# rueberger/MJHMC

Hardware: AMD Instinct MI355X
Metric: particle-steps/sec (ndims x nparticles x L) (higher is better)
Workload: dtype f64 state (ProductOfT: around the f32 matrix-core force)

## Files before the change

### mjhmc_amd/csrc/dense_pot64.hip

```cpp
#include <hip/hip_runtime.h>
#include <stdint.h>

#include <algorithm>

#include "dense_pot.hpp"
#include "dense_pot64_kernels.hpp"
#include "dense_pot_tile.hpp"

namespace mjhmc {

__global__ void pot64_cold_list_kernel(const double* __restrict__ Hflf_in, const double* __restrict__ Hspec_in, int64_t N,
                                       int* __restrict__ list, int* __restrict__ count, const Control* ctl) {
  if (ctl->failed) return;
  const int64_t p = (int64_t)blockIdx.x * blockDim.x + threadIdx.x;
  const double hc = p < N ? Hflf_in[p] : 0.0, hs = p < N ? Hspec_in[p] : 0.0;
  append_cold(list, count, (p < N) && !(hc == hc) && !(hs == hs), p);
}

template <int NB, bool REPLAY, int MODE>
__global__ __launch_bounds__(256, 1) void pot64_jump_kernel(const Pot64JumpArgs a, const PotModel mdl) {
  const PotExperts xp;
#include "dense_pot64_jump.inc"
}

// ... 37 lines not shown
      if (k != 0) {
        a.EX_out[p] = EX0;
        a.EV_out[p] = EV0;
      }
      a.Hflf_out[p] = k == 0 ? H0 : __builtin_nan("");
      a.Hspec_out[p] = k == 1 ? HL : __builtin_nan("");
    }
    __syncthreads();
    if (__syncthreads_or(sh.s.move[c] != 0)) {
      const size_t roff = (size_t)p * (128 * NB) + 32 * NB * w + 4 * NB * h;
      VTile<NB> v;
      Tile<NB> g;
      pot64_finish<NB, REPLAY, kModeMJHMC, true>(a, sh, p, alive, roff, w, c, h, v, g);
      __syncthreads();
    }
  }
  if (any_bad) {
    a.ctl->failed = 1;
    a.ctl->failed_iter = a.iter;
  }
  __shared__ unsigned tally[4];
  if (threadIdx.x < 4) tally[threadIdx.x] = 0;
  __syncthreads();
  if (n0) atomicAdd(&tally[0], n0);
  if (n1) atomicAdd(&tally[1], n1);
  if (n2) atomicAdd(&tally[2], n2);
  if (n3) atomicAdd(&tally[3], n3);
  __syncthreads();
  if (threadIdx.x < 4 && tally[threadIdx.x]) atomicAdd(&a.stats[threadIdx.x], (unsigned long long)tally[threadIdx.x]);
}

static int resident_cus64() {
  int dev = 0, cus = 0;
  (void)hipGetDevice(&dev);
  (void)hipDeviceGetAttribute(&cus, hipDeviceAttributeMultiprocessorCount, dev);
  return std::max(1, cus);
}

int pot64_scratch_workgroups() { return resident_cus64(); }

template <int NB, int MODE>
static void launch64_mode(const Pot64JumpArgs& a, const PotModel& mdl, unsigned grid, hipStream_t st, const PotGenerated* gen) {
  const bool replay = MODE == kModeControl ? (a.runif && a.noise) : (a.rexp && a.noise);
  if (gen) pot_launch_generated(gen->jump64[MODE][replay ? 1 : 0], grid, st, a, mdl, gen->lin);
  else if (replay) hipLaunchKernelGGL((pot64_jump_kernel<NB, true, MODE>), dim3(grid), dim3(256), 0, st, a, mdl);
  else hipLaunchKernelGGL((pot64_jump_kernel<NB, false, MODE>), dim3(grid), dim3(256), 0, st, a, mdl);
}

template <int NB>
static void launch64_nb(const Pot64JumpArgs& a, const PotModel& mdl, hipStream_t st, const PotGenerated* gen) {
  const int cus = resident_cus64();
  if (a.mode == kModeMJHMC) {
    if (a.iter == 0 || a.rescan) {
      (void)hipMemsetAsync(std::min(a.cold_count, std::min(a.next_count, a.zero_count)), 0, 3 * sizeof(int), st);
      hipLaunchKernelGGL(pot64_cold_list_kernel, dim3((unsigned)((a.N + 255) / 256)), dim3(256), 0, st, a.Hflf_in, a.Hspec_in,
                         a.N, a.cold_list, a.cold_count, (const Control*)a.ctl);
    }
    const unsigned grid = (unsigned)std::min<int64_t>(2 * a.ntiles, cus);
    launch64_mode<NB, kModeMJHMC>(a, mdl, grid, st, gen);
    const unsigned fgrid = (unsigned)std::min<int64_t>(a.ntiles, 4 * cus);
    if (a.rexp && a.noise) hipLaunchKernelGGL((pot64_decide_kernel<NB, true>), dim3(fgrid), dim3(256), 0, st, a);
    else hipLaunchKernelGGL((pot64_decide_kernel<NB, false>), dim3(fgrid), dim3(256), 0, st, a);
  } else {
    const unsigned grid = (unsigned)std::min<int64_t>(a.ntiles, cus);
    if (a.mode == kModeCT) launch64_mode<NB, kModeCT>(a, mdl, grid, st, gen);
    else launch64_mode<NB, kModeControl>(a, mdl, grid, st, gen);
  }
}

void pot64_launch_jump(const Pot64JumpArgs& a, const PotModel& mdl, hipStream_t st, const PotGenerated* gen) {
  if (mdl.dim == 128) launch64_nb<1>(a, mdl, st, gen);
  else if (mdl.dim == 256) launch64_nb<2>(a, mdl, st, gen);
  else launch64_nb<4>(a, mdl, st, gen);
}

#ifdef POT_STAMPS
}
extern "C" int mjhmc_pot64_stamps(unsigned long long* out) {
  return (int)hipMemcpyFromSymbol(out, HIP_SYMBOL(mjhmc::g_pot_stamp), sizeof(mjhmc::g_pot_stamp));
}
extern "C" int mjhmc_pot64_item_stamps(unsigned long long* out) {
  return (int)hipMemcpyFromSymbol(out, HIP_SYMBOL(mjhmc::g_pot_istamp), sizeof(mjhmc::g_pot_istamp));
}
namespace mjhmc {
#endif

}
```

### mjhmc_amd/csrc/dense_pot64_jump.inc

```
  __shared__ Shared64<NB> sh;
  if (a.ctl->failed) return;
  const int lane = threadIdx.x & 63, w = threadIdx.x >> 6, c = lane & 31, h = lane >> 5;
  const int ncold = MODE == kModeMJHMC ? *a.cold_count : 0;
  const int64_t nft = (ncold + kP - 1) / kP;
  if ((int64_t)blockIdx.x >= nft + a.ntiles) return;
  if (MODE == kModeMJHMC && blockIdx.x == 0 && threadIdx.x == 0) {
    *a.zero_count = 0;
    if (ncold) atomicAdd(&a.stats[3], (unsigned long long)ncold << 32);
  }
  __shared__ unsigned tally[5];
  if (threadIdx.x < 5) tally[threadIdx.x] = 0;
  AReg<NB> ar;
  areg_load<NB>(mdl, w, c, h, ar);
  stage_bias<NB>(mdl, sh.s);
  const Work<NB> wk = work_of<NB>(a.scratch, blockIdx.x, w, lane);
  for (int64_t item = blockIdx.x; item < nft + a.ntiles; item += gridDim.x) {
    const bool inverse = item < nft;
    [[maybe_unused]] const int istamp_item = (int)(item / gridDim.x) & 15;
    auto column_of = [&](int64_t it) -> int64_t {
      if (it < nft) {
        const int64_t slot = it * kP + c;
        return a.cold_list[slot < ncold ? slot : ncold - 1];
      }
      return (it - nft) * kP + c;
    };
    Tile<NB> g;
    VTile<NB> v;
    float exl = 0.f;
    double EVL;
    {
      const int64_t p = column_of(item);
      POT_ISTAMP(0);
      staged_start<NB>(sh.s, wk, a.X_in, a.V_in, a.G_in, p, w, c, h, g, v, inverse);
      POT_ISTAMP(1);
      EVL = pot64_trajectory<NB>(mdl, xp, ar, sh, w, c, h, lane, wk, g, v, a.L, a.eps, a.chalf, &exl);
      POT_ISTAMP(2);
    }
    int64_t item_again = item;
    asm volatile("" : "+s"(item_again));
    const int64_t p = column_of(item_again);
    const bool alive = p < a.N;
    const size_t roff = (size_t)p * (128 * NB) + 32 * NB * w + 4 * NB * h;
    if (!inverse) staged_end_x<NB>(sh.s, wk, a.X_out, p, w, c, h);
    POT_ISTAMP(3);
    const double EXL = (double)exl;
    const double HL = EXL + EVL;
    if (inverse) {
      if (w == 0 && h == 0) a.Hwork[p] = HL;
      __syncthreads();
      POT_ISTAMP(4);
      continue;
    }

    if constexpr (MODE == kModeMJHMC) {
      if (w == 0 && h == 0) {
        a.EX_out[p] = EXL;
        a.EV_out[p] = EVL;
      }
      staged_end_vg<NB>(sh.s, a.V_out, a.G_out, p, w, c, h, v, g);
      POT_ISTAMP(4);
      continue;
    }

    if (w == 0 && h == 0) {
      const int64_t pp = alive ? p : 0;
      const uint32_t pid = (uint32_t)(a.first_pid + pp);
      const double EX0 = a.EX_in[p], EV0 = a.EV_in[p];
      const double H0 = EX0 + EV0;
      double best = 0.0;
      bool bad = false, gate = false;
      const int k = pot64_decide<REPLAY, MODE>(a, H0, HL, 0.0, pp, pid, best, bad, gate);
      if (bad && alive) tally[4] = 1;
      a.dwell[p] = best;
      a.dwell_ring[p] = best;
      a.trans[p] = (uint8_t)k;
      sh.s.move[c] = k | (gate ? 4 : 0);
      {
        unsigned long long b0, b1, b2, b3 = 0ull;
        if constexpr (MODE == kModeControl) {
          b0 = __ballot(alive && k == 3);
          b1 = __ballot(alive && k == 2);
          b2 = __ballot(alive && gate);
          b3 = __ballot(alive && k == 1);
        } else {
          b0 = __ballot(alive && k == 0);
          b1 = __ballot(alive && k == 1);
          b2 = __ballot(alive && k == 2);
        }
        if (c == 0) {
          if (b0) atomicAdd(&tally[0], (unsigned)__popcll(b0));
          if (b1) atomicAdd(&tally[1], (unsigned)__popcll(b1));
          if (b2) atomicAdd(&tally[2], (unsigned)__popcll(b2));
          if (b3) atomicAdd(&tally[3], (unsigned)__popcll(b3));
        }
      }
      const bool took_L = MODE == kModeControl ? (k & 1) : (k == 0);
      a.EX_out[p] = took_L ? EXL : EX0;
      a.EV_out[p] = took_L ? EVL : EV0;
      a.Hflf_out[p] = __builtin_nan("");
    }
    __syncthreads();
    pot64_finish<NB, REPLAY, MODE, false>(a, sh, p, alive, roff, w, c, h, v, g);
    __syncthreads();
    POT_ISTAMP(4);
  }
  __syncthreads();
  if (threadIdx.x == 0 && tally[4]) {
    a.ctl->failed = 1;
    a.ctl->failed_iter = a.iter;
  }
  if (threadIdx.x < 4 && tally[threadIdx.x]) atomicAdd(&a.stats[threadIdx.x], (unsigned long long)tally[threadIdx.x]);
```

### mjhmc_amd/csrc/dense_pot64_kernels.hpp

```cpp
#pragma once
#ifndef __HIPCC_RTC__
#include <hip/hip_runtime.h>
#endif
#include <stdint.h>

#include "dense_pot.hpp"
#include "dense_pot_tile.hpp"

namespace mjhmc {

template <int NB>
struct DVecN;
template <>
struct DVecN<1> {
  using type = double;
};
template <>
struct DVecN<2> {
  using type = __attribute__((ext_vector_type(2))) double;
};
template <>
struct DVecN<4> {
  using type = __attribute__((ext_vector_type(4))) double;
};
// ... 31 lines not shown
template <int NB>
struct Shared64 {
  Shared<NB> s;
  double red64[4][kP];
  double zn[128 * NB];
  f32x4 park[kPark / 2][256];
};

template <int NB>
struct Work {
  static constexpr int PB = NB == 1 ? 8 : 16;
  static constexpr int PQ = NB * 8 / PB;
  static constexpr unsigned kArea = 16u * PQ * 64u * PB;
  __amdgpu_buffer_rsrc_t rs;
  unsigned voff;
  static constexpr unsigned xb = 0;
  static constexpr unsigned vb = 4 * kArea;
};
template <int NB>
__device__ __forceinline__ Work<NB> work_of(double* scratch, unsigned wg, int w, int lane) {
  Work<NB> k;
  char* base = (char*)scratch + (size_t)wg * (8 * Work<NB>::kArea);
  k.rs = __builtin_amdgcn_make_buffer_rsrc((void*)base, 0, 8 * Work<NB>::kArea, 0x00020000);
  k.voff = (unsigned)w * Work<NB>::kArea + (unsigned)lane * Work<NB>::PB;
  return k;
}
using uvec4 = __attribute__((ext_vector_type(4))) unsigned;
using uvec2 = __attribute__((ext_vector_type(2))) unsigned;
using f64x2 = __attribute__((ext_vector_type(2))) double;
template <int NB>
__device__ __forceinline__ typename DVecN<NB>::type wk_load(const Work<NB>& k, unsigned area, int q) {
  if constexpr (NB == 1) {
    return __builtin_bit_cast(double, __builtin_amdgcn_raw_buffer_load_b64(k.rs, k.voff, area + (unsigned)q * 512u, 0));
  } else if constexpr (NB == 2) {
    return __builtin_bit_cast(f64x2, __builtin_amdgcn_raw_buffer_load_b128(k.rs, k.voff, area + (unsigned)q * 1024u, 0));
  } else {
    const f64x2 lo = __builtin_bit_cast(f64x2, __builtin_amdgcn_raw_buffer_load_b128(k.rs, k.voff, area + (unsigned)q * 2048u, 0));
    const f64x2 hi = __builtin_bit_cast(f64x2, __builtin_amdgcn_raw_buffer_load_b128(k.rs, k.voff, area + (unsigned)q * 2048u + 1024u, 0));
    typename DVecN<4>::type v;
    v[0] = lo[0];
    v[1] = lo[1];
    v[2] = hi[0];
    v[3] = hi[1];
    return v;
  }
}
template <int NB>
__device__ __forceinline__ void wk_store(const Work<NB>& k, unsigned area, int q, const typename DVecN<NB>::type& v) {
  if constexpr (NB == 1) {
    __builtin_amdgcn_raw_buffer_store_b64(__builtin_bit_cast(uvec2, v), k.rs, k.voff, area + (unsigned)q * 512u, 0);
  } else if constexpr (NB == 2) {
    __builtin_amdgcn_raw_buffer_store_b128(__builtin_bit_cast(uvec4, v), k.rs, k.voff, area + (unsigned)q * 1024u, 0);
  } else {
    f64x2 lo, hi;
    lo[0] = v[0];
    lo[1] = v[1];
    hi[0] = v[2];
    hi[1] = v[3];
    __builtin_amdgcn_raw_buffer_store_b128(__builtin_bit_cast(uvec4, lo), k.rs, k.voff, area + (unsigned)q * 2048u, 0);
    __builtin_amdgcn_raw_buffer_store_b128(__builtin_bit_cast(uvec4, hi), k.rs, k.voff, area + (unsigned)q * 2048u + 1024u, 0);
  }
}

template <int NB>
struct PieceOf {
  using type = uvec4;
};
template <>
struct PieceOf<1> {
  using type = unsigned long long;
};
template <int NB>
struct Stage {
  using P = typename PieceOf<NB>::type;
  static constexpr int PB = sizeof(P);
  static constexpr int RB = 1024 * NB;
  static constexpr int RP = RB / PB;
  static constexpr int K = 32 * RP / 256;
  static constexpr int KB = K < 16 ? K : 16;
};
__device__ __forceinline__ unsigned stage_addr(int row, int piece, int pb, int rb) {
  return (unsigned)(row * rb + ((piece ^ (row & 15)) * pb));
}
template <int NB>
__device__ __forceinline__ void stage_rows_in(const double* rows, int64_t p, char* img) {
  using S = Stage<NB>;
  using P = typename S::P;
  const int t = threadIdx.x;
#pragma unroll 1
  for (int i0 = 0; i0 < S::K; i0 += S::KB) {
    P buf[S::KB];
#pragma unroll
    for (int i = 0; i < S::KB; ++i) {
      const int k = (i0 + i) * 256 + t, row = k / S::RP, piece = k % S::RP;
      const int64_t pr = __shfl((long long)p, row);
      buf[i] = *reinterpret_cast<const P*>(reinterpret_cast<const char*>(rows) + (size_t)pr * S::RB + (size_t)piece * S::PB);
    }
#pragma unroll
    for (int i = 0; i < S::KB; ++i) {
      const int k = (i0 + i) * 256 + t, row = k / S::RP, piece = k % S::RP;
      *reinterpret_cast<P*>(img + stage_addr(row, piece, S::PB, S::RB)) = buf[i];
    }
  }
}
template <int NB>
__device__ __forceinline__ void stage_rows_out(double* rows, int64_t p, const char* img) {
  using S = Stage<NB>;
  using P = typename S::P;
  const int t = threadIdx.x;
#pragma unroll 1
  for (int i0 = 0; i0 < S::K; i0 += S::KB) {
#pragma unroll
    for (int i = 0; i < S::KB; ++i) {
      const int k = (i0 + i) * 256 + t, row = k / S::RP, piece = k % S::RP;
      const int64_t pr = __shfl((long long)p, row);
      *reinterpret_cast<P*>(reinterpret_cast<char*>(rows) + (size_t)pr * S::RB + (size_t)piece * S::PB) =
          *reinterpret_cast<const P*>(img + stage_addr(row, piece, S::PB, S::RB));
    }
  }
}
template <int NB>
__device__ __forceinline__ typename DVecN<NB>::type stage_get(const char* img, int w, int c, int h, int q) {
  using S = Stage<NB>;
  const int first = (8 * NB * (32 * w + acc_row(q, h))) / S::PB;
  if constexpr (NB == 4) {
    const f64x2 lo = *reinterpret_cast<const f64x2*>(img + stage_addr(c, first, S::PB, S::RB));
    const f64x2 hi = *reinterpret_cast<const f64x2*>(img + stage_addr(c, first + 1, S::PB, S::RB));
    typename DVecN<4>::type v;
    v[0] = lo[0];
    v[1] = lo[1];
    v[2] = hi[0];
    v[3] = hi[1];
    return v;
  } else {
    return *reinterpret_cast<const typename DVecN<NB>::type*>(img + stage_addr(c, first, S::PB, S::RB));
  }
}
template <int NB>
__device__ __forceinline__ void stage_put(char* img, int w, int c, int h, int q, const typename DVecN<NB>::type& v) {
  using S = Stage<NB>;
  const int first = (8 * NB * (32 * w + acc_row(q, h))) / S::PB;
  if constexpr (NB == 4) {
    f64x2 lo, hi;
    lo[0] = v[0];
    lo[1] = v[1];
    hi[0] = v[2];
    hi[1] = v[3];
    *reinterpret_cast<f64x2*>(img + stage_addr(c, first, S::PB, S::RB)) = lo;
    *reinterpret_cast<f64x2*>(img + stage_addr(c, first + 1, S::PB, S::RB)) = hi;
  } else {
    *reinterpret_cast<typename DVecN<NB>::type*>(img + stage_addr(c, first, S::PB, S::RB)) = v;
  }
}
template <int NB>
__device__ __forceinline__ char* stage_image(Shared<NB>& s) {
  static_assert(sizeof(s.pub) == 32 * Stage<NB>::RB, "the staging image is the two B-operand images");
  return reinterpret_cast<char*>(&s.pub[0][0]);
}

template <int NB>
struct VTile {
  double b[NB][16];
};

template <int NB, int NKICK>
__device__ __forceinline__ void kick_drift_pass(const Work<NB>& wk, const Tile<NB>& g, VTile<NB>& v, double c, double eps,
                                                PubWave<NB>* pub0, int w, int lane) {
  using DV = typename DVecN<NB>::type;
  DV xa[4], xb[4];
  auto load4 = [&](int q4, DV(&x)[4]) {
#pragma unroll
    for (int qq = 0; qq < 4; ++qq) x[qq] = wk_load<NB>(wk, wk.xb, 4 * q4 + qq);
  };
  auto kick4 = [&](int q4) {
#pragma unroll
    for (int qq = 0; qq < 4; ++qq) {
      const int q = 4 * q4 + qq;
#pragma unroll
      for (int r = 0; r < NB; ++r) {
        const double t = c * (double)g.b[r][q];
        double vv = v.b[r][q];
        vv = vv + t;
        if constexpr (NKICK == 2) vv = vv + t;
        v.b[r][q] = vv;
      }
    }
  };
  auto drift4 = [&](int q4, DV(&x)[4]) {
    f32x4 px[NB];
#pragma unroll
    for (int qq = 0; qq < 4; ++qq) {
      const int q = 4 * q4 + qq;
#pragma unroll
      for (int r = 0; r < NB; ++r) {
        const double xx = dget<NB>(x[qq], r) + eps * v.b[r][q];
        dset<NB>(x[qq], r, xx);
        px[r][qq] = (float)xx;
      }
      wk_store<NB>(wk, wk.xb, q, x[qq]);
    }
    if constexpr (NB == 4) {
      unsigned off = ((wk.voff >> 1) & 0xFFFFC000u) | (wk.voff & 0x3FFu);
      asm volatile("" : "+v"(off));
      char* img = reinterpret_cast<char*>(pub0) + off;
#pragma unroll
      for (int r = 0; r < NB; ++r) *reinterpret_cast<f32x4*>(img + (size_t)(r * 4 + q4) * 1024) = px[r];
    } else {
#pragma unroll
      for (int r = 0; r < NB; ++r) pub0[w].v[r][q4][lane] = px[r];
    }
  };
  load4(0, xa);
  load4(1, xb);
  __builtin_amdgcn_sched_barrier(0);
  kick4(0);
  drift4(0, xa);
  __builtin_amdgcn_sched_barrier(0);
  load4(2, xa);
  __builtin_amdgcn_sched_barrier(0);
  kick4(1);
  drift4(1, xb);
  __builtin_amdgcn_sched_barrier(0);
  load4(3, xb);
  __builtin_amdgcn_sched_barrier(0);
  kick4(2);
  drift4(2, xa);
  __builtin_amdgcn_sched_barrier(0);
  kick4(3);
  drift4(3, xb);
}

template <int NB>
__device__ __forceinline__ double closing_kick(const Tile<NB>& g, VTile<NB>& v, double c) {
  double s = 0.0;
#pragma unroll
  for (int q = 0; q < 16; ++q)
#pragma unroll
    for (int r = 0; r < NB; ++r) {
      const double vv = v.b[r][q] + c * (double)g.b[r][q];
      v.b[r][q] = vv;
      s = s + vv * vv;
    }
  return s;
}

template <int NB, class SH>
__device__ __forceinline__ double column_sum(SH& sh, int w, int c, int h, double part) {
  const double both = swap32_sum(part);
  if (h == 0) sh.red64[w][c] = both;
  __syncthreads();
  const double tot = sh.red64[0][c] + sh.red64[1][c] + sh.red64[2][c] + sh.red64[3][c];
  __syncthreads();
  return tot;
}

template <int NB>
__device__ __forceinline__ void staged_start(Shared<NB>& s, const Work<NB>& wk, const double* xin, const double* vin,
                                             const double* gin, int64_t p, int w, int c, int h, Tile<NB>& g, VTile<NB>& v,
                                             bool neg) {
  char* img = stage_image<NB>(s);
  stage_rows_in<NB>(xin, p, img);
  __syncthreads();
#pragma unroll
  for (int q = 0; q < 16; ++q) wk_store<NB>(wk, wk.xb, q, stage_get<NB>(img, w, c, h, q));
  __syncthreads();
  stage_rows_in<NB>(gin, p, img);
  __syncthreads();
#pragma unroll
  for (int q = 0; q < 16; ++q) {
    const typename DVecN<NB>::type gg = stage_get<NB>(img, w, c, h, q);
#pragma unroll
    for (int r = 0; r < NB; ++r) g.b[r][q] = (float)dget<NB>(gg, r);
  }
  __syncthreads();
  stage_rows_in<NB>(vin, p, img);
  __syncthreads();
#pragma unroll
  for (int q = 0; q < 16; ++q) {
    const typename DVecN<NB>::type vv = stage_get<NB>(img, w, c, h, q);
#pragma unroll
    for (int r = 0; r < NB; ++r) v.b[r][q] = neg ? -dget<NB>(vv, r) : dget<NB>(vv, r);
  }
  __syncthreads();
}

template <int NB>
__device__ __forceinline__ void staged_end_x(Shared<NB>& s, const Work<NB>& wk, double* xout, int64_t p, int w, int c, int h) {
  char* img = stage_image<NB>(s);
#pragma unroll
  for (int q = 0; q < 16; ++q) stage_put<NB>(img, w, c, h, q, wk_load<NB>(wk, wk.xb, q));
  __syncthreads();
  stage_rows_out<NB>(xout, p, img);
  __syncthreads();
}
template <int NB>
__device__ __forceinline__ void staged_end_vg(Shared<NB>& s, double* vout, double* gout, int64_t p, int w, int c, int h,
                                              const VTile<NB>& v, const Tile<NB>& g) {
  using DV = typename DVecN<NB>::type;
  char* img = stage_image<NB>(s);
#pragma unroll
  for (int q = 0; q < 16; ++q) {
    DV vv;
#pragma unroll
    for (int r = 0; r < NB; ++r) dset<NB>(vv, r, v.b[r][q]);
    stage_put<NB>(img, w, c, h, q, vv);
  }
  __syncthreads();
  stage_rows_out<NB>(vout, p, img);
  __syncthreads();
#pragma unroll
  for (int q = 0; q < 16; ++q) {
    DV gg;
#pragma unroll
    for (int r = 0; r < NB; ++r) dset<NB>(gg, r, (double)g.b[r][q]);
    stage_put<NB>(img, w, c, h, q, gg);
  }
  __syncthreads();
  stage_rows_out<NB>(gout, p, img);
  __syncthreads();
}

template <int NB, class XP>
__device__ __forceinline__ double pot64_trajectory(const PotModel& mdl, const XP& xp, AReg<NB>& ar, Shared64<NB>& sh, int w, int c, int h,
                                                   int lane, const Work<NB>& wk, Tile<NB>& g, VTile<NB>& v, int L, double eps,
                                                   double chalf, float* ex) {
  PubWave<NB>* pub0 = sh.s.pub[0];
  kick_drift_pass<NB, 1>(wk, g, v, chalf, eps, pub0, w, lane);
  for (int s = 0; s < L; ++s) {
    [[maybe_unused]] const int stamp_slot = s;
    POT_STAMP(0);
    if constexpr (NB == 4) {
#pragma unroll
      for (int k = 0; k < kPark / 2; ++k) {
        f64x2 two;
        two[0] = v.b[NB - 1][15 - 2 * k];
        two[1] = v.b[NB - 1][14 - 2 * k];
        sh.park[k][threadIdx.x] = __builtin_bit_cast(f32x4, two);
      }
    }
    pot_gradient_published<NB>(mdl, xp, ar, sh.s, w, c, h, lane, g, s == L - 1, ex, s);
    if constexpr (NB == 4) {
#pragma unroll
      for (int k = 0; k < kPark / 2; ++k) {
        const f64x2 two = __builtin_bit_cast(f64x2, sh.park[k][threadIdx.x]);
        v.b[NB - 1][15 - 2 * k] = two[0];
        v.b[NB - 1][14 - 2 * k] = two[1];
      }
#pragma unroll
      for (int r = 0; r < NB; ++r)
#pragma unroll
        for (int q = 0; q < 16; ++q) use_here(v.b[r][q]);
    }
    POT_STAMP(6);
    if (s < L - 1) kick_drift_pass<NB, 2>(wk, g, v, chalf, eps, pub0, w, lane);
    POT_STAMP(7);
  }
  const double part = closing_kick<NB>(g, v, chalf);
  return column_sum<NB>(sh, w, c, h, part) / 2.0;
}


template <int NB>
struct Finish64Shared {
  struct {
    int move[kP];
  } s;
  double red64[4][kP];
  double zn[128 * NB];
};

template <int NB, bool REPLAY, int MODE, bool FIX, class SH>
__device__ __forceinline__ void pot64_finish(const Pot64JumpArgs& a, SH& sh, int64_t p, bool alive, size_t roff, int w, int c,
                                             int h, const VTile<NB>& v, const Tile<NB>& g) {
  using DV = typename DVecN<NB>::type;
  const double* xin = a.X_in + roff;
  const double* vin = a.V_in + roff;
  const double* gin = a.G_in + roff;
  double* xo = a.X_out + roff;
  double* vo = a.V_out + roff;
  double* go = a.G_out + roff;
  const int mv = sh.s.move[c];
  const int k = mv & 3;
  bool take, flip, refresh;
  if constexpr (MODE == kModeControl) {
    const bool accept = k & 1, fl = k & 2;
    take = accept;
    flip = accept != fl;
    refresh = (mv & 4) != 0;
  } else {
    take = k == 0;
    flip = (MODE == kModeCT && k == 0) || k == 1;
    refresh = k == 2;
  }
  const bool tile_refreshes = __ballot(refresh) != 0ull;
  if (!FIX || !take) {
#pragma unroll
    for (int q = 0; q < 16; ++q) {
      DV gg;
      if (take) {
        if constexpr (!FIX) {
          DV vv;
#pragma unroll
          for (int r = 0; r < NB; ++r) {
            dset<NB>(vv, r, flip ? -v.b[r][q] : v.b[r][q]);
            dset<NB>(gg, r, (double)g.b[r][q]);
          }
          dv_store<NB>(vo, q, vv);
        }
      } else {
        gg = dv_load<NB>(gin, q);
// ... 107 lines not shown
```

### mjhmc_amd/csrc/dense_pot_tile.hpp

```cpp
#pragma once
#ifndef __HIPCC_RTC__
#include <hip/hip_runtime.h>
#endif
#include <stdint.h>

#include "dense_pot.hpp"
#include "timing_variants.hpp"

namespace mjhmc {

using f32x16 = __attribute__((ext_vector_type(16))) float;
using f32x4 = __attribute__((ext_vector_type(4))) float;

constexpr int kP = 32;

__device__ __forceinline__ int acc_row(int q, int h) { return (q & 3) + 8 * (q >> 2) + 4 * h; }

template <int NB>
struct Tile {
  f32x16 b[NB];
};

template <int NB>
struct VecN;
// ... 62 lines not shown
      v[1] = t.b[r][4 * q4 + 1];
      v[2] = t.b[r][4 * q4 + 2];
      v[3] = t.b[r][4 * q4 + 3];
      dst.v[r][q4][lane] = v;
    }
}

template <int NB>
__device__ __forceinline__ void a_chunk_load(const float* mlane, int chunk, typename VecN<NB>::type (&dst)[16]) {
  using V = typename VecN<NB>::type;
  constexpr int DIM = 128 * NB;
  const float* base = mlane + (size_t)(32 * NB * (chunk / NB) + (chunk % NB)) * DIM;
#pragma unroll
  for (int q = 0; q < 16; ++q) dst[q] = *reinterpret_cast<const V*>(base + (size_t)(NB * ((q & 3) + 8 * (q >> 2))) * DIM);
}

template <int NB>
__device__ __forceinline__ typename VecN<NB>::type buf_load(__amdgpu_buffer_rsrc_t r, unsigned voff, unsigned soff) {
  using V = typename VecN<NB>::type;
  if constexpr (NB == 4) return __builtin_bit_cast(V, __builtin_amdgcn_raw_buffer_load_b128(r, voff, soff, 0));
  else if constexpr (NB == 2) return __builtin_bit_cast(V, __builtin_amdgcn_raw_buffer_load_b64(r, voff, soff, 0));
  else return __builtin_bit_cast(V, __builtin_amdgcn_raw_buffer_load_b32(r, voff, soff, 0));
}
template <int NB>
__device__ __forceinline__ __amdgpu_buffer_rsrc_t a_rsrc(const float* M) {
  constexpr int DIM = 128 * NB;
  return __builtin_amdgcn_make_buffer_rsrc((void*)M, 0, DIM * DIM * 4, 0x00020000);
}
template <int NB>
__device__ __forceinline__ void a_chunk_load_buf(__amdgpu_buffer_rsrc_t r, unsigned lane_bytes, int chunk,
                                                 typename VecN<NB>::type (&dst)[16]) {
  constexpr int DIM = 128 * NB;
  const unsigned cbase = (unsigned)(32 * NB * (chunk / NB) + (chunk % NB)) * (unsigned)(DIM * 4);
#pragma unroll
  for (int q = 0; q < 16; ++q) dst[q] = buf_load<NB>(r, lane_bytes, cbase + (unsigned)(NB * ((q & 3) + 8 * (q >> 2)) * DIM * 4));
}

template <int NB>
__device__ __forceinline__ void chunk_mfma(const f32x4* bbase, int chunk, int lane, const typename VecN<NB>::type (&a)[16],
                                           f32x4& bnext, Tile<NB>& acc) {
  constexpr int NG = 16 * NB;
#pragma unroll
  for (int q4 = 0; q4 < 4; ++q4) {
    const f32x4 b4 = bnext;
    const int t = 4 * chunk + q4 + 1;
    bnext = bbase[(size_t)(t < NG ? t : NG - 1) * 64 + lane];
    __builtin_amdgcn_sched_barrier(0);
#pragma unroll
    for (int qq = 0; qq < 4; ++qq) {
#pragma unroll
      for (int r = 0; r < NB; ++r)
        acc.b[r] = __builtin_amdgcn_mfma_f32_32x32x2f32(vget<NB>(a[4 * q4 + qq], r), b4[qq], acc.b[r], 0, 0, 0);
    }
    __builtin_amdgcn_sched_barrier(0);
  }
}

template <int NB>
__device__ __forceinline__ void chunk_mfma_ld(const f32x4* bbase, int chunk, int lane, const typename VecN<NB>::type (&a)[16],
                                              f32x4& bnext, Tile<NB>& acc, __amdgpu_buffer_rsrc_t rs, unsigned lane_bytes,
                                              unsigned cbase, typename VecN<NB>::type (&aload)[16]) {
  constexpr int NG = 16 * NB, DIM = 128 * NB;
#pragma unroll
  for (int q4 = 0; q4 < 4; ++q4) {
    const f32x4 b4 = bnext;
    const int t = 4 * chunk + q4 + 1;
    bnext = bbase[(size_t)(t < NG ? t : NG - 1) * 64 + lane];
    __builtin_amdgcn_sched_barrier(0);
#pragma unroll
    for (int qq = 0; qq < 4; ++qq) {
      const int q = 4 * q4 + qq;
#pragma unroll
      for (int r = 0; r < NB; ++r)
        acc.b[r] = __builtin_amdgcn_mfma_f32_32x32x2f32(vget<NB>(a[q], r), b4[qq], acc.b[r], 0, 0, 0);
      aload[q] = buf_load<NB>(rs, lane_bytes, cbase + (unsigned)(NB * ((q & 3) + 8 * (q >> 2)) * DIM * 4));
      __builtin_amdgcn_sched_barrier(0);
    }
    __builtin_amdgcn_sched_barrier(0);
  }
}

template <int NB>
__device__ __forceinline__ void gemm_dim(const float* __restrict__ M, const float* __restrict__ Mnext, const PubWave<NB>* pub,
                                         int w, int c, int h, int lane, typename VecN<NB>::type (&a0)[16], Tile<NB>& acc) {
  constexpr int DIM = 128 * NB, NCH = 4 * NB;
  const size_t lane_off = (size_t)(4 * NB * h) * DIM + 32 * NB * w + NB * c;
  const unsigned lane_bytes = (unsigned)(lane_off * sizeof(float));
  const __amdgpu_buffer_rsrc_t rM = a_rsrc<NB>(M), rN = a_rsrc<NB>(Mnext);
  const f32x4* bbase = &pub[0].v[0][0][0];
  typename VecN<NB>::type a1[16];
  f32x4 bnext = bbase[lane];
#pragma unroll 1
  for (int chunk = 0; chunk < NCH; chunk += 2) {
    const bool more = chunk + 2 < NCH;
    const int c1 = chunk + 1, c2 = more ? chunk + 2 : 0;
    chunk_mfma_ld<NB>(bbase, chunk, lane, a0, bnext, acc, rM, lane_bytes,
                      (unsigned)(32 * NB * (c1 / NB) + (c1 % NB)) * (unsigned)(DIM * 4), a1);
    chunk_mfma_ld<NB>(bbase, chunk + 1, lane, a1, bnext, acc, more ? rM : rN, lane_bytes,
                      (unsigned)(32 * NB * (c2 / NB) + (c2 % NB)) * (unsigned)(DIM * 4), a0);
  }
}

template <int NB>
struct AReg {
  typename VecN<NB>::type a0[16];
};
template <>
struct AReg<1> {
  float w1[4][16];
  float w2[4][16];
};

template <int NB>
__device__ __forceinline__ void areg_load(const PotModel& mdl, int w, int c, int h, AReg<NB>& ar) {
  if constexpr (NB == 1) {
    const float* m1 = mdl.W1 + (size_t)(4 * h) * 128 + 32 * w + c;
    const float* m2 = mdl.W2T + (size_t)(4 * h) * 128 + 32 * w + c;
#pragma unroll
    for (int chunk = 0; chunk < 4; ++chunk) {
      a_chunk_load<1>(m1, chunk, ar.w1[chunk]);
      a_chunk_load<1>(m2, chunk, ar.w2[chunk]);
    }
  } else {
    a_chunk_load<NB>(mdl.W1 + (size_t)(4 * NB * h) * (128 * NB) + 32 * NB * w + NB * c, 0, ar.a0);
  }
}

template <int NB, bool SECOND>
__device__ __forceinline__ void gemm_any(const PotModel& mdl, AReg<NB>& ar, const PubWave<NB>* pub, int w, int c,
                                         int h, int lane, Tile<NB>& acc) {
  if constexpr (NB == 1) {
    const int kdim = mdl.ndims;
#pragma unroll
    for (int chunk = 0; chunk < 4; ++chunk) {
      const float(&a)[16] = SECOND ? ar.w2[chunk] : ar.w1[chunk];
      const f32x4(*blk)[64] = pub[chunk].v[0];
#pragma unroll
      for (int q4 = 0; q4 < 4; ++q4) {
        if (32 * chunk + 8 * q4 < kdim) {
          const f32x4 b4 = blk[q4][lane];
#pragma unroll
          for (int qq = 0; qq < 4; ++qq)
            acc.b[0] = __builtin_amdgcn_mfma_f32_32x32x2f32(a[4 * q4 + qq], b4[qq], acc.b[0], 0, 0, 0);
        }
      }
    }
  } else {
    gemm_dim<NB>(SECOND ? mdl.W2T : mdl.W1, SECOND ? mdl.W1 : mdl.W2T, pub, w, c, h, lane, ar.a0, acc);
  }
}

template <int NB>
__device__ __forceinline__ void rowvec_load(const float* vec, int w, int h, Tile<NB>& t) {
  using V = typename VecN<NB>::type;
  const float* base = vec + 32 * NB * w;
#pragma unroll
  for (int q = 0; q < 16; ++q) {
    const V v = *reinterpret_cast<const V*>(base + NB * acc_row(q, h));
#pragma unroll
    for (int r = 0; r < NB; ++r) t.b[r][q] = vget<NB>(v, r);
  }
}

__device__ __forceinline__ float half_sum(float s) {
  const auto sw = __builtin_amdgcn_permlane32_swap(__float_as_int(s), __float_as_int(s), false, false);
  return __int_as_float(sw[0]) + __int_as_float(sw[1]);
}

template <int NB>
struct Shared {
  PubWave<NB> pub[2][4];
  float red[2][4][kP];
  int move[kP];
  float cb[128 * NB];
  float zn[128 * NB];
};

template <int NB>
struct FinishShared {
  float red[2][4][kP];
  int move[kP];
  float zn[128 * NB];
};

template <int NB, typename F>
__device__ __forceinline__ void column_normals(const RngKey& key, uint32_t pid, int D, F* zn) {
  const int pair = threadIdx.x;
  if (pair < 64 * NB) {
    double z0, z1;
    normal_pair(key, pid, (uint32_t)pair, z0, z1);
    zn[2 * pair] = 2 * pair < D ? (F)z0 : (F)0;
    zn[2 * pair + 1] = 2 * pair + 1 < D ? (F)z1 : (F)0;
  }
}

template <int NB>
__device__ __forceinline__ void stage_bias(const PotModel& mdl, Shared<NB>& sh) {
  for (int i = threadIdx.x; i < 128 * NB; i += 256) sh.cb[i] = mdl.cb[i];
}


struct PotExperts {
  static constexpr bool kProductOfT = true;
};

template <int NB, class XP>
__device__ __forceinline__ void pot_gradient_published(const PotModel& mdl, const XP& xp, AReg<NB>& ar, Shared<NB>& sh, int w, int c, int h,
                                                       int lane, Tile<NB>& g, bool want_energy, float* energy_out,
                                                       int stamp_slot = 0) {
  __syncthreads();
  POT_STAMP(1);
  Tile<NB> u;
  rowvec_load<NB>(sh.cb, w, h, u);
  gemm_any<NB, false>(mdl, ar, sh.pub[0], w, c, h, lane, u);
  POT_STAMP(2);
  if constexpr (XP::kProductOfT) {
    if (want_energy) {
      using V = typename VecN<NB>::type;
      const float* al = mdl.alpha + 32 * NB * w;
      float s = 0.f;
#pragma unroll
      for (int q = 0; q < 16; ++q) {
        const V a4 = *reinterpret_cast<const V*>(al + NB * acc_row(q, h));
#pragma unroll
        for (int r = 0; r < NB; ++r) s += vget<NB>(a4, r) * logf(1.0f + u.b[r][q] * u.b[r][q]);
      }
      const float part = half_sum(s);
      if (h == 0) sh.red[0][w][c] = part;
    }
#pragma unroll
    for (int r = 0; r < NB; ++r)
#pragma unroll
      for (int q = 0; q < 16; ++q) {
        const float uu = u.b[r][q];
        u.b[r][q] = uu * __builtin_amdgcn_rcpf(1.0f + uu * uu);
      }
  } else {
    if (want_energy) {
      const float part = half_sum(xp.template energy_sum<NB>(u, w, h));
      if (h == 0) sh.red[0][w][c] = part;
    }
    xp.template phi<NB>(u, w, h);
  }
  publish<NB>(sh.pub[1][w], lane, u);
  POT_STAMP(3);
  __syncthreads();
  POT_STAMP(4);
#pragma unroll
  for (int r = 0; r < NB; ++r)
#pragma unroll
    for (int q = 0; q < 16; ++q) g.b[r][q] = 0.f;
  gemm_any<NB, true>(mdl, ar, sh.pub[1], w, c, h, lane, g);
  POT_STAMP(5);
  if (want_energy && energy_out) {
    *energy_out = sh.red[0][0][c] + sh.red[0][1][c] + sh.red[0][2][c] + sh.red[0][3][c];
  }
}

template <int NB, class XP>
__device__ __forceinline__ void pot_gradient(const PotModel& mdl, const XP& xp, AReg<NB>& ar, Shared<NB>& sh, int w, int c, int h,
                                             int lane, const Tile<NB>& x, Tile<NB>& g, bool want_energy,
                                             float* energy_out) {
  [[maybe_unused]] const int stamp_slot = 0;
  POT_STAMP(0);
  publish<NB>(sh.pub[0][w], lane, x);
  pot_gradient_published<NB>(mdl, xp, ar, sh, w, c, h, lane, g, want_energy, energy_out);
}

template <int NB, class SH>
__device__ __forceinline__ float pot_kinetic(SH& sh, int w, int c, int h, const Tile<NB>& v) {
  float s = 0.f;
#pragma unroll
  for (int r = 0; r < NB; ++r)
#pragma unroll
    for (int q = 0; q < 16; ++q) s += v.b[r][q] * v.b[r][q];
  const float part = half_sum(s);
  if (h == 0) sh.red[1][w][c] = part;
  __syncthreads();
  const float tot = (sh.red[1][0][c] + sh.red[1][1][c] + sh.red[1][2][c] + sh.red[1][3][c]) / 2.0f;
  __syncthreads();
  return tot;
}

template <int NB, class XP>
__device__ __forceinline__ void pot_trajectory(const PotModel& mdl, const XP& xp, AReg<NB>& ar, Shared<NB>& sh, int w, int c, int h,
                                               int lane, Tile<NB>& x, Tile<NB>& v, Tile<NB>& g, int L, float eps,
                                               float chalf, float* ex) {
  if (L > 0) {
#pragma unroll
    for (int r = 0; r < NB; ++r)
#pragma unroll
      for (int q = 0; q < 16; ++q) v.b[r][q] = v.b[r][q] + chalf * g.b[r][q];
  }
  for (int s = 0; s < L; ++s) {
#pragma unroll
    for (int r = 0; r < NB; ++r)
#pragma unroll
      for (int q = 0; q < 16; ++q) x.b[r][q] = x.b[r][q] + eps * v.b[r][q];
    pot_gradient<NB>(mdl, xp, ar, sh, w, c, h, lane, x, g, s == L - 1, ex);
    const float ck = s == L - 1 ? chalf : 2.0f * chalf;
#pragma unroll
    for (int r = 0; r < NB; ++r)
#pragma unroll
      for (int q = 0; q < 16; ++q) v.b[r][q] = v.b[r][q] + ck * g.b[r][q];
  }
}

template <int NB>
__device__ __forceinline__ void pot_normals(const RngKey& key, uint32_t pid, int w, int h, int D, Tile<NB>& z) {
#pragma unroll 1
  for (int q = 0; q < 16; ++q) {
    const int d = 32 * NB * w + NB * acc_row(q, h);
    double zz[4] = {0, 0, 0, 0};
    normal_pair(key, pid, (uint32_t)(d >> 1), zz[0], zz[1]);
    if constexpr (NB == 4) normal_pair(key, pid, (uint32_t)((d >> 1) + 1), zz[2], zz[3]);
    if constexpr (NB == 1) {
      z.b[0][q] = d < D ? (float)((d & 1) ? zz[1] : zz[0]) : 0.f;
    } else {
#pragma unroll
      for (int r = 0; r < NB; ++r) z.b[r][q] = d + r < D ? (float)zz[r] : 0.f;
    }
  }
}

}
```

### mjhmc_amd/csrc/timing_variants.hpp

```cpp
#pragma once

#ifdef POT_STAMPS
namespace mjhmc {
static __device__ unsigned long long g_pot_stamp[4][8][8];
}
#define POT_STAMP(I)                                                                                          \
  do {                                                                                                        \
    if (blockIdx.x == 0 && lane == 0) g_pot_stamp[w][stamp_slot & 7][I] = __builtin_readcyclecounter();      \
  } while (0)
namespace mjhmc {
static __device__ unsigned long long g_pot_istamp[4][16][16];
}
#define POT_ISTAMP(I)                                                                                         \
  do {                                                                                                        \
    if (blockIdx.x == 0 && lane == 0 && a.first_pid == 0) {                                                   \
      g_pot_istamp[w][istamp_item][I] = __builtin_readcyclecounter();                                              \
      g_pot_istamp[w][istamp_item][8 + (I)] = __builtin_amdgcn_s_memrealtime();                            \
    }                                                                                                         \
  } while (0)
#else
#define POT_STAMP(I) do { } while (0)
#define POT_ISTAMP(I) do { } while (0)
#endif

#ifdef SIC_STAMPS
namespace mjhmc {
static __device__ unsigned g_sic_stamp[4][8][8];
}
#define SIC_STAMP(RD, I)                                                                                          \
  do {                                                                                                            \
    if (((I) == (SIC_STAMPS) || ((I) == 0 && (RD) == 0)) && blockIdx.x == 0 && lane == 0 && (w & 2) == 0)         \
      sh.stamp[(w & 1) | ((w >> 2) << 1)][RD][I] = (unsigned)__builtin_readcyclecounter();                        \
  } while (0)
#else
#define SIC_STAMP(RD, I) do { } while (0)
#endif

#ifdef ROWS_STAMPS
namespace mjhmc {
static __device__ unsigned long long g_rows_stamp[4][64][16];
}
#define ROWS_STAMP(I)                                                                                                    \
  do {                                                                                                                   \
    if (blockIdx.x == 0 && stamp_on && (threadIdx.x & 63) == 0) g_rows_stamp[threadIdx.x >> 6][stamp_it & 63][I] = __builtin_readcyclecounter(); \
  } while (0)
#else
#define ROWS_STAMP(I) do { } while (0)
#endif
```

Before: 62.14 billion.

## Batch row loads in staged start, keep initial X in registers, defer X write-out

In MJHMC mode, staged_start now issues the gather loads for G, V and X rows in batches held in registers, overlapping global requests with LDS puts. The initial position tile goes straight into registers and feeds the first kick-drift pass without a scratch reload. The X write-out for non-moving particles is folded into a combined V/G/X store after the trajectory. It also adds optional GEMM cycle stamps under POT_STAMPS. The cost is higher register pressure, which could hurt occupancy or cause spills.

```diff
diff --git a/mjhmc_amd/csrc/dense_pot64.hip b/mjhmc_amd/csrc/dense_pot64.hip
--- a/mjhmc_amd/csrc/dense_pot64.hip
+++ b/mjhmc_amd/csrc/dense_pot64.hip
@@ -143,6 +143,9 @@
 extern "C" int mjhmc_pot64_item_stamps(unsigned long long* out) {
   return (int)hipMemcpyFromSymbol(out, HIP_SYMBOL(mjhmc::g_pot_istamp), sizeof(mjhmc::g_pot_istamp));
 }
+extern "C" int mjhmc_pot64_gemm_stamps(unsigned long long* out) {
+  return (int)hipMemcpyFromSymbol(out, HIP_SYMBOL(mjhmc::g_pot_gstamp), sizeof(mjhmc::g_pot_gstamp));
+}
 namespace mjhmc {
 #endif
 
diff --git a/mjhmc_amd/csrc/dense_pot64_jump.inc b/mjhmc_amd/csrc/dense_pot64_jump.inc
--- a/mjhmc_amd/csrc/dense_pot64_jump.inc
+++ b/mjhmc_amd/csrc/dense_pot64_jump.inc
@@ -30,10 +30,13 @@
     double EVL;
     {
       const int64_t p = column_of(item);
+      constexpr bool kXReg = MODE == kModeMJHMC;
+      typename DVecN<NB>::type x0[16];
       POT_ISTAMP(0);
-      staged_start<NB>(sh.s, wk, a.X_in, a.V_in, a.G_in, p, w, c, h, g, v, inverse);
+      if constexpr (kXReg) staged_start<NB>(sh.s, a.X_in, a.V_in, a.G_in, p, w, c, h, g, v, x0, inverse);
+      else staged_start_serial<NB>(sh.s, wk, a.X_in, a.V_in, a.G_in, p, w, c, h, g, v, inverse);
       POT_ISTAMP(1);
-      EVL = pot64_trajectory<NB>(mdl, xp, ar, sh, w, c, h, lane, wk, g, v, a.L, a.eps, a.chalf, &exl);
+      EVL = pot64_trajectory<NB, kXReg>(mdl, xp, ar, sh, w, c, h, lane, wk, g, v, x0, a.L, a.eps, a.chalf, &exl);
       POT_ISTAMP(2);
     }
     int64_t item_again = item;
@@ -41,13 +44,12 @@
     const int64_t p = column_of(item_again);
     const bool alive = p < a.N;
     const size_t roff = (size_t)p * (128 * NB) + 32 * NB * w + 4 * NB * h;
-    if (!inverse) staged_end_x<NB>(sh.s, wk, a.X_out, p, w, c, h);
-    POT_ISTAMP(3);
     const double EXL = (double)exl;
     const double HL = EXL + EVL;
     if (inverse) {
       if (w == 0 && h == 0) a.Hwork[p] = HL;
       __syncthreads();
+      POT_ISTAMP(3);
       POT_ISTAMP(4);
       continue;
     }
@@ -57,10 +59,14 @@
         a.EX_out[p] = EXL;
         a.EV_out[p] = EVL;
       }
-      staged_end_vg<NB>(sh.s, a.V_out, a.G_out, p, w, c, h, v, g);
+      POT_ISTAMP(3);
+      staged_end_vgx<NB>(sh.s, wk, a.V_out, a.G_out, a.X_out, p, w, c, h, v, g);
       POT_ISTAMP(4);
       continue;
     }
+
+    staged_end_x<NB>(sh.s, wk, a.X_out, p, w, c, h);
+    POT_ISTAMP(3);
 
     if (w == 0 && h == 0) {
       const int64_t pp = alive ? p : 0;
diff --git a/mjhmc_amd/csrc/dense_pot64_kernels.hpp b/mjhmc_amd/csrc/dense_pot64_kernels.hpp
--- a/mjhmc_amd/csrc/dense_pot64_kernels.hpp
+++ b/mjhmc_amd/csrc/dense_pot64_kernels.hpp
@@ -137,6 +137,60 @@
 __device__ __forceinline__ unsigned stage_addr(int row, int piece, int pb, int rb) {
   return (unsigned)(row * rb + ((piece ^ (row & 15)) * pb));
 }
+__device__ __forceinline__ int stage_thread() {
+  int t = (int)threadIdx.x;
+  asm volatile("" : "+v"(t));
+  return t;
+}
+template <int NB>
+__device__ __forceinline__ int stage_row_of(int i, int t) {
+  static_assert(256 % Stage<NB>::RP == 0, "a request of the 256 threads covers whole rows");
+  if constexpr (Stage<NB>::RP == 256) return i;
+  else return __builtin_amdgcn_readfirstlane((i * 256 + t) / Stage<NB>::RP);
+}
+__device__ __forceinline__ int64_t column_particle(int64_t p, int row) {
+  const unsigned lo = (unsigned)__builtin_amdgcn_readlane((int)(unsigned)(unsigned long long)p, row);
+  const unsigned hi = (unsigned)__builtin_amdgcn_readlane((int)(unsigned)((unsigned long long)p >> 32), row);
+  return (int64_t)(((unsigned long long)hi << 32) | lo);
+}
+template <int NB, int HALF>
+__device__ __forceinline__ void stage_rows_request(const double* rows, int64_t p, int t, typename Stage<NB>::P (&buf)[Stage<NB>::K / 2]) {
+  using S = Stage<NB>;
+  using P = typename S::P;
+  const unsigned off = (unsigned)(t % S::RP) * S::PB;
+#pragma unroll
+  for (int i = 0; i < S::K / 2; ++i) {
+    const int rw = stage_row_of<NB>(HALF * (S::K / 2) + i, t);
+    const char* row = reinterpret_cast<const char*>(rows) + (size_t)column_particle(p, rw) * S::RB;
+    buf[i] = *reinterpret_cast<const P*>(row + off);
+  }
+}
+template <int NB, int HALF>
+__device__ __forceinline__ void stage_rows_put(char* img, int t, const typename Stage<NB>::P (&buf)[Stage<NB>::K / 2]) {
+  using S = Stage<NB>;
+  using P = typename S::P;
+  const int piece = t % S::RP;
+#pragma unroll
+  for (int i = 0; i < S::K / 2; ++i)
+    *reinterpret_cast<P*>(img + stage_addr(stage_row_of<NB>(HALF * (S::K / 2) + i, t), piece, S::PB, S::RB)) = buf[i];
+}
+template <int NB>
+__device__ __forceinline__ void stage_rows_out(double* rows, int64_t p, const char* img) {
+  using S = Stage<NB>;
+  using P = typename S::P;
+  const int t = stage_thread();
+  const int piece = t % S::RP;
+  const unsigned off = (unsigned)piece * S::PB;
+#pragma unroll 1
+  for (int i0 = 0; i0 < S::K; i0 += S::KB) {
+#pragma unroll
+    for (int i = 0; i < S::KB; ++i) {
+      const int rw = stage_row_of<NB>(i0 + i, t);
+      char* row = reinterpret_cast<char*>(rows) + (size_t)column_particle(p, rw) * S::RB;
+      *reinterpret_cast<P*>(row + off) = *reinterpret_cast<const P*>(img + stage_addr(rw, piece, S::PB, S::RB));
+    }
+  }
+}
 template <int NB>
 __device__ __forceinline__ void stage_rows_in(const double* rows, int64_t p, char* img) {
   using S = Stage<NB>;
@@ -159,7 +213,7 @@
   }
 }
 template <int NB>
-__device__ __forceinline__ void stage_rows_out(double* rows, int64_t p, const char* img) {
+__device__ __forceinline__ void stage_rows_out_serial(double* rows, int64_t p, const char* img) {
   using S = Stage<NB>;
   using P = typename S::P;
   const int t = threadIdx.x;
@@ -218,14 +272,18 @@
   double b[NB][16];
 };
 
-template <int NB, int NKICK>
+template <int NB, int NKICK, bool PRE = false>
 __device__ __forceinline__ void kick_drift_pass(const Work<NB>& wk, const Tile<NB>& g, VTile<NB>& v, double c, double eps,
-                                                PubWave<NB>* pub0, int w, int lane) {
+                                                PubWave<NB>* pub0, int w, int lane,
+                                                const typename DVecN<NB>::type* pre = nullptr) {
   using DV = typename DVecN<NB>::type;
   DV xa[4], xb[4];
   auto load4 = [&](int q4, DV(&x)[4]) {
 #pragma unroll
-    for (int qq = 0; qq < 4; ++qq) x[qq] = wk_load<NB>(wk, wk.xb, 4 * q4 + qq);
+    for (int qq = 0; qq < 4; ++qq) {
+      if constexpr (PRE) x[qq] = pre[4 * q4 + qq];
+      else x[qq] = wk_load<NB>(wk, wk.xb, 4 * q4 + qq);
+    }
   };
   auto kick4 = [&](int q4) {
 #pragma unroll
@@ -310,7 +368,58 @@
 }
 
 template <int NB>
-__device__ __forceinline__ void staged_start(Shared<NB>& s, const Work<NB>& wk, const double* xin, const double* vin,
+__device__ __forceinline__ void staged_start(Shared<NB>& s, const double* xin, const double* vin, const double* gin, int64_t p,
+                                             int w, int c, int h, Tile<NB>& g, VTile<NB>& v,
+                                             typename DVecN<NB>::type (&x)[16], bool neg) {
+  using P = typename Stage<NB>::P;
+  char* img = stage_image<NB>(s);
+  P g0[Stage<NB>::K / 2], g1[Stage<NB>::K / 2], v0[Stage<NB>::K / 2], v1[Stage<NB>::K / 2], x0[Stage<NB>::K / 2], x1[Stage<NB>::K / 2];
+  const int t = stage_thread();
+  stage_rows_request<NB, 0>(gin, p, t, g0);
+  stage_rows_request<NB, 1>(gin, p, t, g1);
+  __builtin_amdgcn_sched_barrier(0);
+  stage_rows_put<NB, 0>(img, t, g0);
+  __builtin_amdgcn_sched_barrier(0);
+  stage_rows_request<NB, 0>(vin, p, t, v0);
+  __builtin_amdgcn_sched_barrier(0);
+  stage_rows_put<NB, 1>(img, t, g1);
+  __builtin_amdgcn_sched_barrier(0);
+  stage_rows_request<NB, 1>(vin, p, t, v1);
+  __builtin_amdgcn_sched_barrier(0);
+  __syncthreads();
+#pragma unroll
+  for (int q = 0; q < 16; ++q) {
+    const typename DVecN<NB>::type gg = stage_get<NB>(img, w, c, h, q);
+#pragma unroll
+    for (int r = 0; r < NB; ++r) g.b[r][q] = (float)dget<NB>(gg, r);
+  }
+  __syncthreads();
+  stage_rows_put<NB, 0>(img, t, v0);
+  __builtin_amdgcn_sched_barrier(0);
+  stage_rows_request<NB, 0>(xin, p, t, x0);
+  __builtin_amdgcn_sched_barrier(0);
+  stage_rows_put<NB, 1>(img, t, v1);
+  __syncthreads();
+#pragma unroll
+  for (int q = 0; q < 16; ++q) {
+    const typename DVecN<NB>::type vv = stage_get<NB>(img, w, c, h, q);
+#pragma unroll
+    for (int r = 0; r < NB; ++r) v.b[r][q] = neg ? -dget<NB>(vv, r) : dget<NB>(vv, r);
+  }
+  __syncthreads();
+  stage_rows_put<NB, 0>(img, t, x0);
+  __builtin_amdgcn_sched_barrier(0);
+  stage_rows_request<NB, 1>(xin, p, t, x1);
+  __builtin_amdgcn_sched_barrier(0);
+  stage_rows_put<NB, 1>(img, t, x1);
+  __syncthreads();
+#pragma unroll
+  for (int q = 0; q < 16; ++q) x[q] = stage_get<NB>(img, w, c, h, q);
+  __syncthreads();
+}
+
+template <int NB>
+__device__ __forceinline__ void staged_start_serial(Shared<NB>& s, const Work<NB>& wk, const double* xin, const double* vin,
                                              const double* gin, int64_t p, int w, int c, int h, Tile<NB>& g, VTile<NB>& v,
                                              bool neg) {
   char* img = stage_image<NB>(s);
@@ -339,18 +448,19 @@
   __syncthreads();
 }
 
+
 template <int NB>
 __device__ __forceinline__ void staged_end_x(Shared<NB>& s, const Work<NB>& wk, double* xout, int64_t p, int w, int c, int h) {
   char* img = stage_image<NB>(s);
 #pragma unroll
   for (int q = 0; q < 16; ++q) stage_put<NB>(img, w, c, h, q, wk_load<NB>(wk, wk.xb, q));
   __syncthreads();
-  stage_rows_out<NB>(xout, p, img);
-  __syncthreads();
-}
-template <int NB>
-__device__ __forceinline__ void staged_end_vg(Shared<NB>& s, double* vout, double* gout, int64_t p, int w, int c, int h,
-                                              const VTile<NB>& v, const Tile<NB>& g) {
+  stage_rows_out_serial<NB>(xout, p, img);
+  __syncthreads();
+}
+template <int NB>
+__device__ __forceinline__ void staged_end_vgx(Shared<NB>& s, const Work<NB>& wk, double* vout, double* gout, double* xout,
+                                               int64_t p, int w, int c, int h, const VTile<NB>& v, const Tile<NB>& g) {
   using DV = typename DVecN<NB>::type;
   char* img = stage_image<NB>(s);
 #pragma unroll
@@ -360,6 +470,11 @@
     for (int r = 0; r < NB; ++r) dset<NB>(vv, r, v.b[r][q]);
     stage_put<NB>(img, w, c, h, q, vv);
   }
+  __builtin_amdgcn_sched_barrier(0);
+  DV x[16];
+#pragma unroll
+  for (int q = 0; q < 16; ++q) x[q] = wk_load<NB>(wk, wk.xb, q);
+  __builtin_amdgcn_sched_barrier(0);
   __syncthreads();
   stage_rows_out<NB>(vout, p, img);
   __syncthreads();
@@ -373,14 +488,21 @@
   __syncthreads();
   stage_rows_out<NB>(gout, p, img);
   __syncthreads();
-}
-
-template <int NB, class XP>
+#pragma unroll
+  for (int q = 0; q < 16; ++q) stage_put<NB>(img, w, c, h, q, x[q]);
+  __syncthreads();
+  stage_rows_out<NB>(xout, p, img);
+  __syncthreads();
+}
+
+template <int NB, bool XREG, class XP>
 __device__ __forceinline__ double pot64_trajectory(const PotModel& mdl, const XP& xp, AReg<NB>& ar, Shared64<NB>& sh, int w, int c, int h,
-                                                   int lane, const Work<NB>& wk, Tile<NB>& g, VTile<NB>& v, int L, double eps,
+                                                   int lane, const Work<NB>& wk, Tile<NB>& g, VTile<NB>& v,
+                                                   const typename DVecN<NB>::type (&x0)[16], int L, double eps,
                                                    double chalf, float* ex) {
   PubWave<NB>* pub0 = sh.s.pub[0];
-  kick_drift_pass<NB, 1>(wk, g, v, chalf, eps, pub0, w, lane);
+  if constexpr (XREG) kick_drift_pass<NB, 1, true>(wk, g, v, chalf, eps, pub0, w, lane, x0);
+  else kick_drift_pass<NB, 1>(wk, g, v, chalf, eps, pub0, w, lane);
   for (int s = 0; s < L; ++s) {
     [[maybe_unused]] const int stamp_slot = s;
     POT_STAMP(0);
diff --git a/mjhmc_amd/csrc/dense_pot_tile.hpp b/mjhmc_amd/csrc/dense_pot_tile.hpp
--- a/mjhmc_amd/csrc/dense_pot_tile.hpp
+++ b/mjhmc_amd/csrc/dense_pot_tile.hpp
@@ -168,7 +168,8 @@
 
 template <int NB>
 __device__ __forceinline__ void gemm_dim(const float* __restrict__ M, const float* __restrict__ Mnext, const PubWave<NB>* pub,
-                                         int w, int c, int h, int lane, typename VecN<NB>::type (&a0)[16], Tile<NB>& acc) {
+                                         int w, int c, int h, int lane, typename VecN<NB>::type (&a0)[16], Tile<NB>& acc,
+                                         [[maybe_unused]] int gstamp = -1) {
   constexpr int DIM = 128 * NB, NCH = 4 * NB;
   const size_t lane_off = (size_t)(4 * NB * h) * DIM + 32 * NB * w + NB * c;
   const unsigned lane_bytes = (unsigned)(lane_off * sizeof(float));
@@ -176,6 +177,7 @@
   const f32x4* bbase = &pub[0].v[0][0][0];
   typename VecN<NB>::type a1[16];
   f32x4 bnext = bbase[lane];
+  POT_GSTAMP(gstamp, 0);
 #pragma unroll 1
   for (int chunk = 0; chunk < NCH; chunk += 2) {
     const bool more = chunk + 2 < NCH;
@@ -184,6 +186,7 @@
                       (unsigned)(32 * NB * (c1 / NB) + (c1 % NB)) * (unsigned)(DIM * 4), a1);
     chunk_mfma_ld<NB>(bbase, chunk + 1, lane, a1, bnext, acc, more ? rM : rN, lane_bytes,
                       (unsigned)(32 * NB * (c2 / NB) + (c2 % NB)) * (unsigned)(DIM * 4), a0);
+    POT_GSTAMP(gstamp, chunk / 2 + 1);
   }
 }
 
@@ -214,7 +217,7 @@
 
 template <int NB, bool SECOND>
 __device__ __forceinline__ void gemm_any(const PotModel& mdl, AReg<NB>& ar, const PubWave<NB>* pub, int w, int c,
-                                         int h, int lane, Tile<NB>& acc) {
+                                         int h, int lane, Tile<NB>& acc, [[maybe_unused]] int gstamp = -1) {
   if constexpr (NB == 1) {
     const int kdim = mdl.ndims;
 #pragma unroll
@@ -232,7 +235,7 @@
       }
     }
   } else {
-    gemm_dim<NB>(SECOND ? mdl.W2T : mdl.W1, SECOND ? mdl.W1 : mdl.W2T, pub, w, c, h, lane, ar.a0, acc);
+    gemm_dim<NB>(SECOND ? mdl.W2T : mdl.W1, SECOND ? mdl.W1 : mdl.W2T, pub, w, c, h, lane, ar.a0, acc, gstamp);
   }
 }
 
@@ -298,7 +301,7 @@
   POT_STAMP(1);
   Tile<NB> u;
   rowvec_load<NB>(sh.cb, w, h, u);
-  gemm_any<NB, false>(mdl, ar, sh.pub[0], w, c, h, lane, u);
+  gemm_any<NB, false>(mdl, ar, sh.pub[0], w, c, h, lane, u, POT_GSTAMP_OF(stamp_slot, 0));
   POT_STAMP(2);
   if constexpr (XP::kProductOfT) {
     if (want_energy) {
@@ -336,7 +339,7 @@
   for (int r = 0; r < NB; ++r)
 #pragma unroll
     for (int q = 0; q < 16; ++q) g.b[r][q] = 0.f;
-  gemm_any<NB, true>(mdl, ar, sh.pub[1], w, c, h, lane, g);
+  gemm_any<NB, true>(mdl, ar, sh.pub[1], w, c, h, lane, g, POT_GSTAMP_OF(stamp_slot, 1));
   POT_STAMP(5);
   if (want_energy && energy_out) {
     *energy_out = sh.red[0][0][c] + sh.red[0][1][c] + sh.red[0][2][c] + sh.red[0][3][c];
diff --git a/mjhmc_amd/csrc/timing_variants.hpp b/mjhmc_amd/csrc/timing_variants.hpp
--- a/mjhmc_amd/csrc/timing_variants.hpp
+++ b/mjhmc_amd/csrc/timing_variants.hpp
@@ -18,9 +18,20 @@
       g_pot_istamp[w][istamp_item][8 + (I)] = __builtin_amdgcn_s_memrealtime();                            \
     }                                                                                                         \
   } while (0)
+namespace mjhmc {
+constexpr int kPotGemmStep = 10;
+static __device__ unsigned long long g_pot_gstamp[4][2][16];
+}
+#define POT_GSTAMP_OF(SLOT, G) ((SLOT) == kPotGemmStep ? (G) : -1)
+#define POT_GSTAMP(G, I)                                                                                      \
+  do {                                                                                                        \
+    if (blockIdx.x == 0 && lane == 0 && (G) >= 0) g_pot_gstamp[w][G][(I) & 15] = __builtin_readcyclecounter(); \
+  } while (0)
 #else
 #define POT_STAMP(I) do { } while (0)
 #define POT_ISTAMP(I) do { } while (0)
+#define POT_GSTAMP_OF(SLOT, G) (-1)
+#define POT_GSTAMP(G, I) do { } while (0)
 #endif
 
 #ifdef SIC_STAMPS
```

Result: no change. 62.54 billion (median of 6 runs) (+0.6%).
